# actuday6418/ray-tracer-s8

Measured on AMD Instinct MI355X. Metric: Mrays/sec @ 4K/8spp 1024-sphere, higher is better.
Workload: dtype f32

## Files before the change

ray_tracer_s8_amd/csrc/rt_kernel.hip.h:

```cpp
#pragma once
#include <hip/hip_runtime.h>
#include <type_traits>
#include <stdint.h>

#include "rt_consts.h"
#include "rt_cull.h"

namespace rtk {

#ifndef RT_MINWAVES
#define RT_MINWAVES 4
#endif
#ifndef RT_MINWAVES_TRAV
#define RT_MINWAVES_TRAV 4
#endif
#ifndef RT_MINWAVES_LTREE
#define RT_MINWAVES_LTREE 4
#endif
#ifndef RT_MINWAVES_CULL
#define RT_MINWAVES_CULL 5
#endif
#ifndef RT_STEPS_PER_CHECK_X
#define RT_STEPS_PER_CHECK_X 16
#endif
#ifndef RT_QUEUE_TAKE_MIN
#define RT_QUEUE_TAKE_MIN 4
#endif
#ifndef RT_BF2
#define RT_BF2 1
#endif
#ifndef RT_CULL_FLUSH_MIN
#define RT_CULL_FLUSH_MIN 1
#endif
#ifndef RT_MINWAVES_QTRAV
#define RT_MINWAVES_QTRAV 5
#endif
#ifndef RT_STEPS_PER_CHECK
#define RT_STEPS_PER_CHECK 8
#endif
#ifndef RT_STEPS_PER_CHECK_LTREE
#define RT_STEPS_PER_CHECK_LTREE 8
#endif
#ifndef RT_STEPS_PER_CHECK_Q
#define RT_STEPS_PER_CHECK_Q 16
#endif
#ifndef RT_LT_PARTIAL
#define RT_LT_PARTIAL 40
#endif
#ifndef RT_LT_EAGER
#define RT_LT_EAGER 12
#endif

constexpr uint32_t SLOT_FREE = 0x80000000u;
struct WaveQ {
    uint32_t cnt[SLOTS_MAX];
    uint32_t cost_acc[2];
    uint32_t cost_strip[2];
};
static_assert(sizeof(WaveQ) == 144, "WaveQ layout (rt_plan.h: LDS_LIMIT leaves 3 KiB of static LDS)");
constexpr uint32_t SLOT_UNIT_BITS = 13;
struct WaveStage {
    int left[STAGE_TILES + 1];
    uint32_t dst_lo[STAGE_TILES + 1], dst_hi[STAGE_TILES + 1];
};

struct StripDesc {
    uint64_t seed;
    uint8_t* rgb;
    float* f32;
    float* acc;
    uint32_t y0;
    uint32_t pad;
};

struct KParams {
    uint32_t W, H, Hs;
    uint32_t upp, depth;
    uint32_t spp_all, s_begin, gap;
    uint32_t acc_out;
    uint32_t n_sph, n_sph_pad;
    uint32_t n_tri;
    uint32_t chunk;
    uint32_t n_chunks;
    uint32_t flags;
    uint32_t path32;
    uint32_t lds_cand_off;
    uint32_t lds_path_off;
    uint32_t lds_rr_off;
    uint32_t lds_stack_off;
    uint32_t lds_cmp_off;
    uint32_t lds_stage_off;
    uint32_t n_strips;
    uint32_t tiles_x, tiles_per_strip;
    uint32_t tiles_total;
    uint32_t tiles_big;
    uint32_t sub_shift;
    uint32_t n_tiles;
    uint32_t n_slots;
    uint32_t grp;
    uint32_t grp_magic;
    uint32_t slot_stride;
    uint32_t commit_slots;
    uint32_t spp_magic;
    uint32_t slotu_magic;
    float* ring;
    float org[3], llc[3], hor[3], ver[3];
    float lens_radius, focus_distance;
    float lens_u[3], lens_v[3];
    float u_den, v_den;
    float t_min, t_max;
    float spp_f;
    float spp_rcp;
    const float4* geom_pk;
    const float4* geom_px;
    const float4* geom;
    const float4* mat;
    const float* emis;
    const float* tri;
    const float4* tri_box;
    const float4* trav;
    const uint4* travq;
    const float4* geom_r;
    float q_base[3], q_step[3], q_rstep[3];
    uint32_t root_ref;
    uint32_t maxl;
    uint32_t list16;
    uint32_t stack_lds;
    uint32_t ovf_stride;
    uint32_t* stack_ovf;
    const uint32_t* big;
    uint32_t n_big;
    float r_slack;
    float tri_k, tri_diag, tri_es, tri_e;
    uint32_t refill_eighths;
    uint32_t n_internal;
    uint32_t lds_node_off;
    const float4* bvh_nodes;
    const uint32_t* leaf_of;
    const uint32_t* world_rank;
    unsigned long long* strip_cost;
    unsigned long long* counters;
    unsigned long long* queue;
    StripDesc strips[MAX_BATCH];
    uint32_t plain;
};

struct V3 {
    float x, y, z;
};
__device__ __forceinline__ V3 mk(float x, float y, float z) { return V3{x, y, z}; }
__device__ __forceinline__ V3 operator+(V3 a, V3 b) { return {a.x + b.x, a.y + b.y, a.z + b.z}; }
__device__ __forceinline__ V3 operator-(V3 a, V3 b) { return {a.x - b.x, a.y - b.y, a.z - b.z}; }
__device__ __forceinline__ V3 operator*(float s, V3 a) { return {s * a.x, s * a.y, s * a.z}; }
__device__ __forceinline__ V3 operator*(V3 a, float s) { return {a.x * s, a.y * s, a.z * s}; }
template <class P>
__device__ __forceinline__ V3 lens_offset(const P& p, float x1, float x2) {
    return mk(x1 * p.lens_u[0] + x2 * p.lens_v[0], x1 * p.lens_u[1] + x2 * p.lens_v[1], x1 * p.lens_u[2] + x2 * p.lens_v[2]);
}
template <bool NEG_OK = false>
__device__ __forceinline__ float sqrt_rn(float x) {
#ifdef RT_IEEE_SQRT_PLAIN
    return __builtin_sqrtf(x);
#else
    const float r = __builtin_amdgcn_rsqf(x);
    float g = x * r, h = 0.5f * r;
    const float e = __builtin_fmaf(-h, g, 0.5f);
    g = __builtin_fmaf(g, e, g);
    h = __builtin_fmaf(h, e, h);
    const float dd = __builtin_fmaf(-g, g, x);
    float y = __builtin_fmaf(dd, h, g);
    const bool odd = ((__float_as_uint(x) & (NEG_OK ? 0x7fffffffu : 0xffffffffu)) - 0x0f800000u) >= (0x7f800000u - 0x0f800000u);
    if (__ballot(odd)) {
        if (odd) {
            asm volatile("" : "+v"(x));
            y = __builtin_sqrtf(x);
        }
    }
    return y;
#endif
}
#define RT_SQRT(x_) sqrt_rn(x_)
#define RT_SQRT_NEG_OK(x_) sqrt_rn<true>(x_)
#define RT_DIV(a_, b_) ((a_) / (b_))
#define RT_HOOK_LT_STEP_LOADS(nd_, ni_, lnodes_)
#define RT_HOOK_LT_STEP_ALU(p0_, p1_, p2_, p3_, oy_)
#define RT_HOOK_LT_STEP_END
#define RT_HOOK_Q_GATHER(t_ref_, cl_, travq_, n_internal_)
#ifdef RT_PROBES
#include "rt_probes.h"
#endif
__device__ __forceinline__ V3 operator/(V3 a, float s) { return {RT_DIV(a.x, s), RT_DIV(a.y, s), RT_DIV(a.z, s)}; }
__device__ __forceinline__ float dot(V3 a, V3 b) { return (a.x * b.x + a.y * b.y) + a.z * b.z; }
__device__ __forceinline__ float vlength(V3 a) { return RT_SQRT(dot(a, a)); }
__device__ __forceinline__ V3 normalize(V3 a) { return a / vlength(a); }
__device__ __forceinline__ bool try_normalize(V3 a, V3& out) {
    float rcp = RT_DIV(1.0f, RT_SQRT(dot(a, a)));
    if (rcp > 0.0f && rcp < __builtin_inff()) {
        out = a * rcp;
        return true;
    }
    return false;
}
__device__ __forceinline__ V3 normalize_or_zero(V3 a) {
// ... 279 lines not shown
    const float lcx = __builtin_fmaf(RT_Q(qa.x, 0), ig.x, cq.x), lcy = __builtin_fmaf(RT_Q(qa.x, 1), ig.y, cq.y), lcz = __builtin_fmaf(RT_Q(qa.y, 0), ig.z, cq.z);
    const float lhx = RT_Q(qa.y, 1), lhy = RT_Q(qa.z, 0), lhz = RT_Q(qa.z, 1);
    const float rcx = __builtin_fmaf(RT_Q(qa.w, 0), ig.x, cq.x), rcy = __builtin_fmaf(RT_Q(qa.w, 1), ig.y, cq.y), rcz = __builtin_fmaf(RT_Q(qb.x, 0), ig.z, cq.z);
    const float rhx = RT_Q(qb.x, 1), rhy = RT_Q(qb.y, 0), rhz = RT_Q(qb.y, 1);
#undef RT_Q
    lmin = __builtin_fmaxf(__builtin_fmaxf(__builtin_fmaf(-lhx, ax, lcx), __builtin_fmaf(-lhy, ay, lcy)), __builtin_fmaf(-lhz, az, lcz));
    lmax = __builtin_fminf(__builtin_fminf(__builtin_fmaf(lhx, ax, lcx), __builtin_fmaf(lhy, ay, lcy)), __builtin_fmaf(lhz, az, lcz));
    rmin_ = __builtin_fmaxf(__builtin_fmaxf(__builtin_fmaf(-rhx, ax, rcx), __builtin_fmaf(-rhy, ay, rcy)), __builtin_fmaf(-rhz, az, rcz));
    rmax_ = __builtin_fminf(__builtin_fminf(__builtin_fmaf(rhx, ax, rcx), __builtin_fmaf(rhy, ay, rcy)), __builtin_fmaf(rhz, az, rcz));
}

__device__ __forceinline__ float cull_bound(float best, V3 o, float r_slack) { return cull_bound(best, o.x, o.y, o.z, r_slack); }
__device__ __forceinline__ float cull_bound_tri(float best, V3 o, float k, float diag, float es, float e) {
    return cull_bound_tri(best, o.x, o.y, o.z, k, diag, es, e);
}

template <int ISECT, bool EXPANDED, int BS = BLOCK, bool STATS = false, bool TRIS = true>
__global__ __launch_bounds__(BS, (ISECT == 5 || ISECT == 6) ? RT_MINWAVES_LTREE : ISECT == 9 ? RT_MINWAVES_TRAV : ISECT >= 7 ? RT_MINWAVES_CULL : ISECT >= 3 ? RT_MINWAVES_QTRAV : ISECT == 2 ? RT_MINWAVES_TRAV : RT_MINWAVES) void rt_tile_kernel(const KParams p) {
    constexpr int BLOCK = BS;
    constexpr bool STREAMED = (ISECT == 1);
    constexpr bool TRAVERSE = (ISECT >= 2);
    constexpr bool QNODES = (ISECT == 3 || ISECT == 4 || ISECT == 7 || ISECT == 8);
    constexpr bool CULL = (ISECT == 6 || ISECT == 7 || ISECT == 8 || ISECT == 9);
    constexpr bool XNODES = (ISECT == 2 || ISECT == 9);
    constexpr bool CAPPED = (ISECT == 4 || ISECT == 8);
    constexpr bool LTREE = (ISECT == 5 || ISECT == 6);
    constexpr uint32_t LB = LTREE ? 0x8000u : LEAF_BIT;
    constexpr bool BFSTEP = LTREE;
    static_assert(TRIS || LTREE, "the sphere-only instantiation exists for the LDS-tree kernels");
    constexpr bool PLAIN_OK = LTREE;
    auto path32 = [&]() -> bool { return !LTREE && p.path32 != 0u; };
    const uint32_t ML = QNODES ? p.maxl : (uint32_t)MAXL_EXACT;
    extern __shared__ __attribute__((aligned(16))) unsigned char lds_raw[];
    __shared__ unsigned long long wg_tiles;
    __shared__ unsigned int wg_lock, wg_drained;
    __shared__ WaveQ wave_q[BS / 64];
    constexpr bool CAN_STAGE = (ISECT >= 1 && ISECT <= 4) || ISECT >= 7;
    __shared__ WaveStage wave_st[CAN_STAGE ? BS / 64 : 1];
    {
        uint32_t* z = reinterpret_cast<uint32_t*>(&wave_q[threadIdx.x >> 6]);
        if ((threadIdx.x & 63u) < SLOTS_MAX) wave_q[threadIdx.x >> 6].cnt[threadIdx.x & 63u] = SLOT_FREE;
        if ((threadIdx.x & 63u) == 0u) {
            wave_q[threadIdx.x >> 6].cost_acc[0] = wave_q[threadIdx.x >> 6].cost_acc[1] = 0u;
            wave_q[threadIdx.x >> 6].cost_strip[0] = wave_q[threadIdx.x >> 6].cost_strip[1] = 0xffffffffu;
        }
        (void)z;
        if (CAN_STAGE && (threadIdx.x & 63u) <= STAGE_TILES) wave_st[threadIdx.x >> 6].left[threadIdx.x & 63u] = -1;
    }
    if (threadIdx.x == 0) {
        wg_tiles = 0ull;
        wg_lock = 0u;
        wg_drained = 0u;
    }
    __syncthreads();
    float4* lgeom = reinterpret_cast<float4*>(lds_raw);
    const float* lgeomf = reinterpret_cast<const float*>(lds_raw);
    float* lrr = reinterpret_cast<float*>(lds_raw + p.lds_rr_off);
    const float4* __restrict__ gsrc = EXPANDED ? p.geom_px : p.geom_pk;
    uint16_t* lcand = reinterpret_cast<uint16_t*>(lds_raw + p.lds_cand_off);
    unsigned char* lpath = lds_raw + p.lds_path_off;

    const int tid = threadIdx.x;
    const int lane = tid & 63;
    const int tid16 = (tid & ~63) | ((tid & 31) << 1) | ((tid >> 5) & 1);

    if (ISECT == 0) {
        for (uint32_t i = tid; i < p.n_sph_pad; i += BLOCK) lgeom[i] = gsrc[i];
        if (EXPANDED)
            for (uint32_t i = tid; i < p.n_sph_pad; i += BLOCK) lrr[i] = p.geom[i].w;
        __syncthreads();
    }

    if (LTREE) {
        float* ln = reinterpret_cast<float*>(lds_raw + p.lds_node_off);
        const uint32_t r0 = lt_r0(p.n_internal);
        for (uint32_t n = tid; n <= p.n_internal; n += BLOCK) {
            float* q = ln + LNODE_DW * n;
            if (n < p.n_internal) {
                const float4 a0 = p.trav[4u * n], a1 = p.trav[4u * n + 1], a2 = p.trav[4u * n + 2], a3 = p.trav[4u * n + 3];
                auto ref16 = [r0](uint32_t r) { return (r & LEAF_BIT) ? (0x8000u | (r & 0x7fffu)) : r0 + r * (uint32_t)LNODE_DW; };
                q[0] = a0.x; q[1] = a1.x; q[2] = a0.x;   q[3] = a2.x; q[4] = a3.x; q[5] = a2.x;
                q[6] = a0.y; q[7] = a1.y; q[8] = a0.y;   q[9] = a2.y; q[10] = a3.y; q[11] = a2.y;
                q[12] = a0.z; q[13] = a1.z; q[14] = a0.z; q[15] = a2.z; q[16] = a3.z; q[17] = a2.z;
                q[18] = __uint_as_float(ref16(__float_as_uint(a0.w)) | (ref16(__float_as_uint(a1.w)) << 16));
            } else {
                const float qn = __builtin_nanf(""), inf = __builtin_inff();
                for (int i = 0; i < 18; i++) q[i] = qn;
                for (int a = 0; a < 3; a++) { q[6 * a] = -inf; q[6 * a + 1] = inf; q[6 * a + 2] = -inf; }
                q[18] = __uint_as_float((r0 + p.n_internal * (uint32_t)LNODE_DW) * 0x10001u);
            }
        }
        float* nanf_ = ln + LNODE_DW * (p.n_internal + 1u);
        for (uint32_t i = tid; i < p.n_sph + p.n_tri + (uint32_t)LNODE_DW; i += BLOCK) nanf_[i] = __builtin_nanf("");
        __syncthreads();
    }
    const float* const lnodes = reinterpret_cast<const float*>(lds_raw + p.lds_node_off) - (LTREE ? (int)lt_r0(p.n_internal) : 0);
    const V3 corg = mk(p.org[0], p.org[1], p.org[2]);
    const V3 llc = mk(p.llc[0], p.llc[1], p.llc[2]);
    const V3 hor = mk(p.hor[0], p.hor[1], p.hor[2]);
    const V3 ver = mk(p.ver[0], p.ver[1], p.ver[2]);
    const bool exact_scan = (p.flags & 1u) != 0;
    const bool use_bvh = (p.flags & 2u) == 0;
    const float KMf = 1.0f - 0x1p-17f;
    const v2f NKM = {-KMf, -KMf};

    const uint32_t wave = (uint32_t)tid >> 6;
#define wq wave_q[wave]
#define wst wave_st[CAN_STAGE ? wave : 0u]
    float* const ring = p.ring + (size_t)(blockIdx.x * (uint32_t)(BLOCK / 64) + wave) * ((size_t)p.n_slots * p.slot_stride * 3u);
    const uint32_t all_free = p.n_slots >= 32u ? 0xffffffffu : (1u << p.n_slots) - 1u;
    uint32_t freem = all_free;
    uint32_t cur_slot = 0;
    uint32_t tile_u = 0, tile_units = 0;
    uint32_t tile_x0 = 0, tile_row = 0, tile_yg = 0;
    uint32_t tile_meta = STAGE_TILES << 16;
    uint64_t tile_seed = 0;
    bool q_drained = false;
    bool have_unit = false, need_ray = false;
    uint32_t useq = 0;
    Rng rng = {0, 0, 0, 0};
    uint32_t depth_left = 0, k = 0;
    V3 o = mk(0, 0, 0), d = mk(0, 0, 0);
    bool bounce = false;
    V3 bn = mk(0, 0, 0);
    float brough = 0.f;
    using Cnt = typename std::conditional<(ISECT >= 2), uint32_t, unsigned long long>::type;
    Cnt n_seg = 0, n_cand = 0, n_fall = 0;
    Cnt n_int = 0;
    Hit h;
    h.idx = -1;
    h.dist = 0.f;
    h.t = 0.f;
    RayAux aux = ray_aux(mk(1.f, 1.f, 1.f), false);
    auto AUX = [&]() -> RayAux { return QNODES ? ray_aux(d, (p.flags & 8u) != 0) : aux; };
    auto far_bound = [&](float best) -> float {
        float b = cull_bound(best, o, p.r_slack);
        if (TRIS && (ISECT == 9 || ISECT == 6) && p.n_tri) b = __builtin_fmaxf(b, cull_bound_tri(best, o, p.tri_k, p.tri_diag, p.tri_es, p.tri_e));
        return b;
    };
    V3 td = mk(0, 0, 0);
    bool in_trav = false;
    uint32_t t_ref = 0, t_sp = 0, t_cnt = 0;
    uint32_t t_head = 0;
    V3 ig = mk(0, 0, 0), cq = mk(0, 0, 0);
    bool qfin = false;
    float t_far = __builtin_inff();
    uint32_t* lc32 = reinterpret_cast<uint32_t*>(lds_raw + p.lds_cand_off);
    uint32_t* lstack = reinterpret_cast<uint32_t*>(lds_raw + p.lds_stack_off);
    uint32_t sgx = 0, sgy = 0, sgz = 0;
    uint16_t* lc16 = reinterpret_cast<uint16_t*>(lds_raw + p.lds_cand_off);
    uint16_t* lstack16 = reinterpret_cast<uint16_t*>(lds_raw + p.lds_stack_off);

    if (BFSTEP) lstack16[tid16] = (uint16_t)(lt_r0(p.n_internal) + p.n_internal * (uint32_t)LNODE_DW);

    auto drain_counters = [&]() {
        const unsigned long long ws = wave_sum(n_seg), wc = wave_sum(n_cand), wf = wave_sum(n_fall);
        const unsigned long long wi = STATS ? wave_sum(n_int) : 0ull;
        if (lane == (int)__builtin_ctzll(__ballot(true))) {
            atomicAdd(&p.counters[0], ws);
            atomicAdd(&p.counters[1], wc);
            atomicAdd(&p.counters[2], wf);
            if (STATS) atomicAdd(&p.counters[3], wi);
        }
        n_seg = n_cand = n_fall = 0;
        n_int = 0;
    };
    const bool staging = CAN_STAGE && p.lds_stage_off != 0xffffffffu;
    unsigned char* const stage_base = lds_raw + (staging ? p.lds_stage_off + wave * (STAGE_TILES * STAGE_TILE_BYTES) : 0u);
    auto decode_tile = [&](uint32_t t, uint32_t& st, uint32_t& x0, uint32_t& row) {
        st = t / p.tiles_per_strip;
        const uint32_t rem = t - st * p.tiles_per_strip;
        row = rem / p.tiles_x;
        x0 = (rem - row * p.tiles_x) << 6;
    };
    auto div_spp = [&](uint32_t q) -> uint32_t { return p.spp_magic ? __umulhi(q, p.spp_magic) : q; };

    TDECL;
    for (;;) {
        WCOUNT(0);
        TSTAMP(5);
        TROUND;
        uint32_t px = 0, pyg = 0;
        if (freem != all_free) {
            __builtin_amdgcn_fence(__ATOMIC_ACQ_REL, "wavefront");
            const bool slot_done = (uint32_t)lane < SLOTS_MAX && (wq.cnt[cold<QNODES>(lane) & (int)(SLOTS_MAX - 1u)] & (SLOT_FREE | ((1u << SLOT_UNIT_BITS) - 1u))) == 0u;
            const uint32_t complete = (uint32_t)__ballot(slot_done);
            const uint32_t n_complete = (uint32_t)__builtin_popcount(complete);
            const bool issue_over = q_drained && tile_u == tile_units;
            if (n_complete >= p.commit_slots || (n_complete != 0u && ((uint32_t)__builtin_popcount(freem) < 2u || issue_over))) {
                WCOUNT(14);
                asm volatile("s_waitcnt vmcnt(0)" ::: "memory");
                auto commit_complete = [&](auto plain_tag) {
                    constexpr bool PLAIN = decltype(plain_tag)::value;
                    const uint32_t n_lanes = PLAIN ? p.n_slots : p.n_slots * p.grp;
                    for (uint32_t l0 = 0; l0 < n_lanes; l0 += 64u) {
                        const uint32_t L = l0 + (uint32_t)lane;
                        const uint32_t slot = (PLAIN || p.grp == 1u) ? L : __umulhi(L, p.grp_magic), g = PLAIN ? 0u : L - slot * p.grp;
                        const bool mine = slot < p.n_slots && ((complete >> (slot & 31u)) & 1u) != 0u;
                        if (__ballot(mine) == 0ull) continue;
                        uint32_t stg = STAGE_TILES, cstrip = 0;
                        bool fin = false;
                        uint32_t pin = 0;
                        if (mine) {
                            const float* sb = ring + __umul24(slot, p.slot_stride) * 3u;
                            const uint32_t hx = ring_load(reinterpret_cast<const uint32_t*>(sb) + 0);
                            const uint32_t hrow = ring_load(reinterpret_cast<const uint32_t*>(sb) + 1);
                            const uint32_t hmeta = ring_load(reinterpret_cast<const uint32_t*>(sb) + 2);
                            const float* r = sb + 3u + g * p.upp * 3u;
                            float sum_r = 0.f, sum_g = 0.f, sum_b = 0.f;
                            cstrip = hmeta & 0xffu;
                            if (!PLAIN && p.s_begin != 0u && g < ((hmeta >> 8) & 0xffu)) {
                                const float* a = p.strips[cstrip].acc + ((size_t)hrow * p.W + hx + g) * 3;
                                sum_r = a[0];
                                sum_g = a[1];
                                sum_b = a[2];
                            }
                            {
                                uint32_t i = 0;
                                auto batch = [&](auto cb_tag) {
                                    constexpr int CB = decltype(cb_tag)::value;
#pragma clang loop unroll(disable)
                                    for (; i + (uint32_t)CB <= p.upp; i += (uint32_t)CB) {
                                        LCOUNT(12);
                                        float c[3 * CB];
#pragma unroll
                                        for (int e = 0; e < 3 * CB; e++) c[e] = ring_load(r + e);
#pragma unroll
                                        for (int e = 0; e < CB; e++) {
                                            sum_r = sum_r + c[3 * e + 0];
                                            sum_g = sum_g + c[3 * e + 1];
                                            sum_b = sum_b + c[3 * e + 2];
                                        }
                                        r += 3 * CB;
                                    }
                                };
                                if (RT_COMMIT_BATCH > 4 && !QNODES) batch(std::integral_constant<int, RT_COMMIT_BATCH>{});
                                batch(std::integral_constant<int, 4>{});
#pragma clang loop unroll(disable)
                                for (; i < p.upp; i++) {
                                    LCOUNT(12);
                                    const float cr = ring_load(r + 0);
                                    const float cg = ring_load(r + 1);
                                    const float cb = ring_load(r + 2);
                                    sum_r = sum_r + cr;
                                    sum_g = sum_g + cg;
                                    sum_b = sum_b + cb;
                                    r += 3;
                                }
                            }
                            if (g < ((hmeta >> 8) & 0xffu)) {
                                float cr_, cg_, cb_;
                                if (PLAIN || p.spp_rcp != 0.0f) {
                                    cr_ = __builtin_sqrtf(sum_r * p.spp_rcp);
                                    cg_ = __builtin_sqrtf(sum_g * p.spp_rcp);
                                    cb_ = __builtin_sqrtf(sum_b * p.spp_rcp);
                                } else {
                                    cr_ = __builtin_sqrtf(sum_r / p.spp_f);
                                    cg_ = __builtin_sqrtf(sum_g / p.spp_f);
                                    cb_ = __builtin_sqrtf(sum_b / p.spp_f);
                                }
                                const uint32_t sidx = hmeta & 0xffu;
                                stg = (hmeta >> 16) & 0xffu;
                                const size_t oidx = ((size_t)hrow * p.W + hx + g) * 3;
                                if (!PLAIN && p.acc_out) {
                                    float* a = p.strips[sidx].acc;
                                    a[oidx + 0] = sum_r;
                                    a[oidx + 1] = sum_g;
                                    a[oidx + 2] = sum_b;
                                }
                                if (!CAN_STAGE || stg == STAGE_TILES) {
                                    uint8_t* orgb = p.strips[sidx].rgb;
                                    orgb[oidx + 0] = f32_as_u8(cr_ * 255.999f);
                                    orgb[oidx + 1] = f32_as_u8(cg_ * 255.999f);
                                    orgb[oidx + 2] = f32_as_u8(cb_ * 255.999f);
                                } else {
                                    uint8_t* sd = stage_base + stg * STAGE_TILE_BYTES + ((hx + g) & 63u) * 3u;
                                    sd[0] = f32_as_u8(cr_ * 255.999f);
                                    sd[1] = f32_as_u8(cg_ * 255.999f);
                                    sd[2] = f32_as_u8(cb_ * 255.999f);
                                    fin = true;
                                }
                                float* of = PLAIN ? nullptr : p.strips[sidx].f32;
                                if (of) {
                                    of[oidx + 0] = cr_;
                                    of[oidx + 1] = cg_;
                                    of[oidx + 2] = cb_;
                                }
                                (void)pin;
                            }
                        }
                        if (!PLAIN && p.strip_cost && mine && g == 0u) {
                            const uint32_t sg = wq.cnt[slot & (SLOTS_MAX - 1u)] >> SLOT_UNIT_BITS;
                            if (cstrip == wq.cost_strip[0]) (void)__hip_atomic_fetch_add(&wq.cost_acc[0], sg, __ATOMIC_RELAXED, __HIP_MEMORY_SCOPE_WAVEFRONT);
                            else if (cstrip == wq.cost_strip[1]) (void)__hip_atomic_fetch_add(&wq.cost_acc[1], sg, __ATOMIC_RELAXED, __HIP_MEMORY_SCOPE_WAVEFRONT);
                            else if (sg) atomicAdd(&p.strip_cost[(blockIdx.x % COST_COPIES) * MAX_BATCH + cstrip], (unsigned long long)sg);
                        }
                        if (CAN_STAGE && __ballot(fin)) {
                            __builtin_amdgcn_fence(__ATOMIC_ACQ_REL, "wavefront");
#pragma unroll
                            for (uint32_t k = 0; k < STAGE_TILES; k++) {
                                const unsigned long long mk = __ballot(fin && stg == k);
                                if (mk == 0ull) continue;
                                const int left = (int)uni((uint32_t)wst.left[k]) - (int)__builtin_popcountll(mk);
                                if (left == 0) {
                                    if (lane < (int)(STAGE_TILE_BYTES / 4)) {
                                        uint32_t* d32 = reinterpret_cast<uint32_t*>(((uintptr_t)uni(wst.dst_hi[k]) << 32) | uni(wst.dst_lo[k]));
// ... 81 lines not shown
                    tile_x0 = uni(tile_x0 + sub);
                    tile_row = uni(tile_row);
                    if (tile_x0 >= p.W) continue;
                    tile_yg = uni(p.strips[tstrip].y0 + tile_row);
                    tile_seed = p.strips[tstrip].seed + (((uint64_t)tile_yg * p.W + tile_x0) * p.spp_all + p.s_begin) * (4ull * PHI);
                    tile_seed = (uint64_t)uni((uint32_t)tile_seed) | ((uint64_t)uni((uint32_t)(tile_seed >> 32)) << 32);
                    const uint32_t npix = min(tw, p.W - tile_x0);
                    tile_units = uni(npix * p.upp);
                    tile_u = 0u;
                    uint32_t tstage = STAGE_TILES;
                    if (staging && npix == 64u) {
                        uint8_t* dst = p.strips[tstrip].rgb + ((size_t)tile_row * p.W + tile_x0) * 3;
                        if ((reinterpret_cast<uintptr_t>(dst) & 3u) == 0) {
                            __builtin_amdgcn_fence(__ATOMIC_ACQ_REL, "wavefront");
                            for (uint32_t k = 0; k < STAGE_TILES; k++)
                                if ((int)uni((uint32_t)wst.left[k]) < 0) {
                                    tstage = k;
                                    break;
                                }
                            if (tstage < STAGE_TILES && lane == 0) {
                                wst.left[tstage] = 64;
                                wst.dst_lo[tstage] = (uint32_t)reinterpret_cast<uintptr_t>(dst);
                                wst.dst_hi[tstage] = (uint32_t)(reinterpret_cast<uintptr_t>(dst) >> 32);
                            }
                            __builtin_amdgcn_fence(__ATOMIC_ACQ_REL, "wavefront");
                        }
                    }
                    tile_meta = uni(tstrip | (tstage << 16));
                }
                bool got = false;
                uint32_t tv = 0;
                bool stall = false;
                {
                    const unsigned long long mask = __ballot(need);
                    const uint32_t want = (uint32_t)__builtin_popcountll(mask);
                    const uint32_t U = p.slot_stride - 1u;
                    const uint32_t k_open = __umulhi(tile_u + U - 1u, p.slotu_magic);
                    const uint32_t n_free = (uint32_t)__builtin_popcount(freem);
                    const uint32_t slot_room = (k_open + n_free) * U - tile_u;
                    const uint32_t take = min(want, min(tile_units - tile_u, slot_room));
                    stall = take < want && take == slot_room;
                    const uint32_t n_new = __umulhi(tile_u + take + U - 1u, p.slotu_magic) - k_open;
                    const uint32_t rank = __builtin_amdgcn_mbcnt_hi((uint32_t)(mask >> 32), __builtin_amdgcn_mbcnt_lo((uint32_t)mask, 0u));
                    got = need && rank < take;
                    tv = tile_u + rank;
                    const uint32_t k = __umulhi(tv, p.slotu_magic);
                    const uint32_t unit = tv - __umul24(k, U);
                    uint32_t m = freem;
                    for (uint32_t i = 0; i + 1u < n_new; i++) m = k > k_open + i ? (m & (m - 1u)) : m;
                    const uint32_t slot = k >= k_open ? (uint32_t)__builtin_ctz(m | 0x80000000u) : cur_slot;
                    if (got) {
                        useq = (slot << 24) | unit;
                        if (unit == 0u) {
                            const uint32_t un = min(U, tile_units - tv);
                            wq.cnt[slot] = un;
                            uint32_t* hdr = reinterpret_cast<uint32_t*>(ring + __umul24(slot, p.slot_stride) * 3u);
                            hdr[0] = tile_x0 + __umul24(k, p.grp);
                            hdr[1] = tile_row;
                            hdr[2] = (tile_meta & 0xffu) | (div_spp(un) << 8) | (tile_meta & 0xff0000u);
                        }
                    }
                    tile_u = uni(tile_u + take);
                    if (n_new) {
                        uint32_t fm = freem;
                        for (uint32_t i = 0; i + 1u < n_new; i++) fm &= fm - 1u;
                        cur_slot = uni((uint32_t)__builtin_ctz(fm));
                        freem = uni(fm & (fm - 1u));
                    }
                }
                TSTAMP(7);
                if (got) {
                    WCOUNT(1);
                    LCOUNT(0);
                    const uint32_t j = div_spp(tv);
                    px = tile_x0 + j;
                    pyg = tile_yg;
                    rng = seed_state(tile_seed + (uint64_t)(tv + __umul24(j, p.gap)) * (4ull * PHI));
                    have_unit = true;
                    need_ray = true;
                    bounce = false;
                    need = false;
                }
                if (stall) { LCOUNT(14); break; }
            }
        }
        const bool active = have_unit;
        if (!active) { LCOUNT(13); }
        TSTAMP(0);
        if (active && need_ray) {
            float x1, x2, sm;
            WCOUNT(2);
            for (;;) {
                WCOUNT(3);
                LCOUNT(1);
                x1 = uniform_m1_1(rng);
                x2 = uniform_m1_1(rng);
                sm = x1 * x1 + x2 * x2;
                if (bounce ? !(sm >= 1.0f) : (sm <= 1.0f)) break;
            }
            V3 xdir, pre, fallback;
            LCOUNT(2);
            if (bounce) {
                LCOUNT(3);
                const float factor = 2.0f * RT_SQRT(1.0f - sm);
                const V3 us = mk(x1 * factor, x2 * factor, 1.0f - 2.0f * sm);
                const V3 diffuse_dir = us + bn;
                const V3 glossy_dir = d - (2.0f * dot(d, bn)) * bn;
                pre = diffuse_dir + brough * (glossy_dir - diffuse_dir);
                fallback = bn;
            } else {
                LCOUNT(4);
                const V3 offset = lens_offset(p, x1, x2);
                const float u = ((float)px + gen_range_01(rng)) / p.u_den;
                const float v = ((float)(p.H - pyg - 1) + gen_range_01(rng)) / p.v_den;
                const V3 dir0 = normalize_or_zero(llc + u * hor + v * ver - corg);
                const V3 d1 = normalize(dir0);
                const V3 focal_point = corg + p.focus_distance * d1;
                o = corg + offset;
                pre = focal_point - o;
                fallback = mk(0.f, 0.f, 0.f);
                depth_left = p.depth;
                k = 0;
            }
            if (!try_normalize(pre, xdir)) xdir = fallback;
            d = normalize(xdir);
            need_ray = false;
            bounce = false;
        }
        TSTAMP(1);
        const bool wave_busy = __ballot(active) != 0ull || freem != all_free || !q_drained || tile_u != tile_units;
        if (STREAMED) {
            if (!__syncthreads_or(wave_busy ? 1 : 0)) break;
        } else {
            if (!wave_busy) break;
        }

        if (active && !in_trav) {
            h.idx = -1;
            aux = ray_aux(d, (p.flags & 8u) != 0);
            if (!TRAVERSE) td = 2.0f * d;
            n_seg++;
            if (QNODES) {
                const V3 og = mk((o.x - p.q_base[0]) * p.q_rstep[0], (o.y - p.q_base[1]) * p.q_rstep[1], (o.z - p.q_base[2]) * p.q_rstep[2]);
                ig = mk(p.q_step[0] * aux.inv.x, p.q_step[1] * aux.inv.y, p.q_step[2] * aux.inv.z);
                cq = mk(-(og.x * ig.x), -(og.y * ig.y), -(og.z * ig.z));
                const float big = 0x1p100f, tiny = 0x1p-60f;
                const float ax = __builtin_fabsf(ig.x), ay = __builtin_fabsf(ig.y), az = __builtin_fabsf(ig.z);
                qfin = aux.finite && ax < big && ay < big && az < big && ax > tiny && ay > tiny && az > tiny &&
                       __builtin_fabsf(og.x) < 0x1p18f && __builtin_fabsf(og.y) < 0x1p18f && __builtin_fabsf(og.z) < 0x1p18f;
            }
            if (LTREE) {
                aux.finite = aux.finite && __builtin_fabsf(o.x) < __builtin_inff() && __builtin_fabsf(o.y) < __builtin_inff() &&
                             __builtin_fabsf(o.z) < __builtin_inff();
                sgx = aux.sx ? 1u : 0u;
                sgy = aux.sy ? 1u : 0u;
                sgz = aux.sz ? 1u : 0u;
            }
            if (CULL) {
                t_far = __builtin_inff();
                for (uint32_t j = 0; j < p.n_big; j++) {
                    const uint32_t prim = p.big[j];
                    float t;
                    bool hit;
                    if (!TRIS || prim < p.n_sph) {
                        const float4 g = RT_SPHERE_REC(p, prim);
                        hit = exact_sphere(o, 2.0f * d, mk(g.x, g.y, g.z), g.w, p.t_min, p.t_max, t);
                    } else {
                        hit = exact_triangle(o, d, p.tri + 9 * (size_t)(prim - p.n_sph), p.t_min, p.t_max, t);
                    }
                    if (hit)
                        consider_if<true>(h, (int)prim, o, d, t, [&]() { return bvh_reaches(p.bvh_nodes, p.leaf_of[prim], o, AUX()); }, p.leaf_of);
                }
                if (h.idx >= 0) t_far = far_bound(h.dist);
            }
            if (TRAVERSE) {
                t_ref = p.root_ref;
                t_sp = BFSTEP ? 1u : 0u;
                t_cnt = 0;
                in_trav = (p.n_sph + p.n_tri) > 0;
            }
        }
        if constexpr (TRAVERSE) {
            auto root_test = [&](uint32_t i) {
                    LCOUNT(6);
                    const uint32_t prim = LTREE ? (uint32_t)lc16[i * BLOCK + tid16] & 0x7fffu
                                          : p.list16 ? (uint32_t)lc16[i * BLOCK + tid16] : lc32[i * BLOCK + tid];
                    float t;
                    if (!TRIS || prim < p.n_sph) {
                        const float4 g = RT_SPHERE_REC(p, prim);
                        if (exact_sphere(o, 2.0f * d, mk(g.x, g.y, g.z), g.w, p.t_min, p.t_max, t)) {
                            if (QNODES)
                                consider_if<CULL>(h, (int)prim, o, d, t, [&]() {
                                    if (!qfin || (p.n_sph + p.n_tri) == 1) return true;
                                    const float4 s = at32(p.geom_r, prim);
                                    return intersects_aabb_finite(o, AUX(), make_float4(s.x - s.w, s.y - s.w, s.z - s.w, 0.f),
                                                                  make_float4(s.x + s.w, s.y + s.w, s.z + s.w, 0.f));
                                }, p.leaf_of);
                            else if (CULL)
                                consider<1>(h, (int)prim, o, d, t, aux, p.bvh_nodes, p.leaf_of);
                            else
                                consider<0>(h, (int)prim, o, d, t, aux, p.bvh_nodes, p.leaf_of);
                        }
                    } else {
                        if (exact_triangle(o, d, p.tri + 9 * (size_t)(prim - p.n_sph), p.t_min, p.t_max, t)) {
                            if (QNODES)
                                consider_if(h, (int)prim, o, d, t,
                                            [&]() { return !qfin || bvh_reaches(p.bvh_nodes, p.leaf_of[prim], o, AUX()); });
                            else if (CULL)
                                consider<1>(h, (int)prim, o, d, t, aux, p.bvh_nodes, p.leaf_of);
                            else
                                consider<0>(h, (int)prim, o, d, t, aux, p.bvh_nodes, p.leaf_of);
                        }
                    }
            };
            auto flush = [&]() {
                if (BFSTEP) n_cand += t_cnt - t_head;
#pragma clang loop unroll(disable)
                for (uint32_t i = BFSTEP ? t_head : 0u; i < t_cnt; i++) root_test(i);
                t_cnt = 0;
                if (BFSTEP) t_head = 0;
                if (CULL && h.idx >= 0) t_far = far_bound(h.dist);
            };
            auto flush_one = [&]() {
                n_cand++;
                root_test(t_head);
                t_head++;
                if (t_head == t_cnt) t_head = t_cnt = 0;
                if (CULL && h.idx >= 0) t_far = far_bound(h.dist);
            };

            constexpr bool COMPACT = XNODES;
            auto flush_c = [&](bool want) {
                const uint32_t cnt = want ? t_cnt : 0u;
                uint32_t excl = 0, total = 0;
#pragma unroll
                for (int b = 0; b < 4; b++) {
                    const unsigned long long m = __ballot(((cnt >> b) & 1u) != 0);
                    excl += (uint32_t)__builtin_amdgcn_mbcnt_hi((uint32_t)(m >> 32), __builtin_amdgcn_mbcnt_lo((uint32_t)m, 0u)) << b;
                    total += (uint32_t)__builtin_popcountll(m) << b;
                }
                const unsigned long long act = __ballot(true);
                const uint32_t n_act = (uint32_t)__builtin_popcountll(act);
                const uint32_t rank = (uint32_t)__builtin_amdgcn_mbcnt_hi((uint32_t)(act >> 32), __builtin_amdgcn_mbcnt_lo((uint32_t)act, 0u));
                uint32_t* const w_pref = reinterpret_cast<uint32_t*>(lds_raw + p.lds_cmp_off) + (tid >> 6) * 256;
                float* const w_dist = reinterpret_cast<float*>(w_pref + 64);
                float* const w_root = reinterpret_cast<float*>(w_pref + 128);
                uint32_t* const w_hit = w_pref + 192;
                w_pref[rank] = excl | ((uint32_t)lane << 16);
                __builtin_amdgcn_fence(__ATOMIC_ACQ_REL, "wavefront");
                int best_k = -1;
                float best_t = 0.f;
                auto own_prim = [&](uint32_t k) -> uint32_t {
                    return p.list16 ? (uint32_t)lc16[k * BLOCK + tid16] : lc32[k * BLOCK + tid];
                };
                for (uint32_t base = 0; base < total; base += n_act) {
                    const uint32_t j = base + rank;
                    const bool valid = j < total;
                    uint32_t R = 0, ent = w_pref[0];
                    if (valid) {
#pragma unroll
                        for (uint32_t stp = 32; stp > 0; stp >>= 1) {
                            const uint32_t c = R + stp;
                            if (c < n_act) {
                                const uint32_t e = w_pref[c];
                                if ((e & 0xffffu) <= j) { R = c; ent = e; }
                            }
                        }
                    }
                    const uint32_t L = ent >> 16, slot = j - (ent & 0xffffu);
                    const V3 ro = mk(__shfl(o.x, (int)L, 64), __shfl(o.y, (int)L, 64), __shfl(o.z, (int)L, 64));
                    const V3 rd = mk(__shfl(d.x, (int)L, 64), __shfl(d.y, (int)L, 64), __shfl(d.z, (int)L, 64));
                    bool hit = false;
                    float t = 0.f, dist = 0.f;
                    if (valid) {
                        LCOUNT(6);
                        const uint32_t ot = ((uint32_t)tid & ~63u) | L;
                        const uint32_t ot16 = (ot & ~63u) | ((ot & 31u) << 1) | ((ot >> 5) & 1u);
                        const uint32_t prim = p.list16 ? (uint32_t)lc16[slot * BLOCK + ot16] : lc32[slot * BLOCK + ot];
                        if (prim < p.n_sph) {
                            const float4 g = RT_SPHERE_REC(p, prim);
                            hit = exact_sphere(ro, 2.0f * rd, mk(g.x, g.y, g.z), g.w, p.t_min, p.t_max, t);
                        } else {
                            hit = exact_triangle(ro, rd, p.tri + 9 * (size_t)(prim - p.n_sph), p.t_min, p.t_max, t);
                        }
                        if (hit) {
                            const V3 pp = ro + t * rd;
                            dist = vlength(pp - ro);
                        }
                    }
                    w_dist[rank] = dist;
                    w_root[rank] = t;
                    w_hit[rank] = hit ? 1u : 0u;
                    __builtin_amdgcn_fence(__ATOMIC_ACQ_REL, "wavefront");
                    if (cnt) {
                        const uint32_t k0 = excl > base ? excl : base, k1 = min(excl + cnt, base + n_act);
#pragma clang loop unroll(disable)
                        for (uint32_t k = k0; k < k1; k++) {
                            if (!w_hit[k - base]) continue;
                            const float dk = w_dist[k - base];
                            bool take = best_k < 0 ? (h.idx < 0 || h.dist > dk) : (h.dist > dk);
                            if (CULL && !take && h.dist == dk && (best_k >= 0 || h.idx >= 0)) {
                                const uint32_t cur = best_k >= 0 ? own_prim((uint32_t)best_k) : (uint32_t)h.idx;
                                take = p.leaf_of[own_prim(k - excl)] < p.leaf_of[cur];
                            }
                            if (take) {
                                h.dist = dk;
                                best_k = (int)(k - excl);
                                best_t = w_root[k - base];
                            }
                        }
                    }
                    __builtin_amdgcn_fence(__ATOMIC_ACQ_REL, "wavefront");
                }
                if (best_k >= 0) {
                    h.idx = (int)own_prim((uint32_t)best_k);
                    h.t = best_t;
                }
                if (want) t_cnt = 0;
                if (CULL && want && h.idx >= 0) t_far = far_bound(h.dist);
            };
            auto push = [&](uint32_t v) {
                if (LTREE) lstack16[t_sp * BLOCK + tid16] = (uint16_t)v;
                else if (!CAPPED || t_sp < p.stack_lds) lstack[t_sp * BLOCK + tid] = v;
                else p.stack_ovf[(size_t)(t_sp - p.stack_lds) * p.ovf_stride + (blockIdx.x * BLOCK + tid)] = v;
                t_sp++;
            };
            auto pop = [&]() -> uint32_t {
                --t_sp;
                if (LTREE) return (uint32_t)lstack16[t_sp * BLOCK + tid16];
                if (!CAPPED || t_sp < p.stack_lds) return lstack[t_sp * BLOCK + tid];
                return p.stack_ovf[(size_t)(t_sp - p.stack_lds) * p.ovf_stride + (blockIdx.x * BLOCK + tid)];
            };
            if constexpr (BFSTEP) {
            const uint32_t DONE = lt_r0(p.n_internal) + p.n_internal * (uint32_t)LNODE_DW;
            constexpr int STEPS = RT_STEPS_PER_CHECK_LTREE;
            static_assert(MAXL_LTREE > STEPS, "the leaf list must take a block of appends");
            constexpr uint32_t SLOT = (uint32_t)BLOCK * 2u;
            typedef __attribute__((address_space(3))) unsigned char lds_byte;
            typedef __attribute__((address_space(3))) uint16_t lds_u16;
            const uint32_t lds0 = (uint32_t)(uintptr_t)(lds_byte*)lds_raw;
            const uint32_t stack0_a = lds0 + p.lds_stack_off + (uint32_t)tid16 * 2u;
            const uint32_t list0_m = lds0 + p.lds_cand_off + (uint32_t)tid16 * 2u - SLOT;
            uint32_t top_a = 0, cnt_m = 0;
            auto lds16 = [&](uint32_t a) -> lds_u16& { return *(lds_u16*)(uintptr_t)a; };
            auto step = [&](auto slow_tag) {
                constexpr bool SLOW = decltype(slow_tag)::value;
                static_assert(SLOT == 0x800u, "leaf flag 0x8000 >> 4 must be one slot");
                const uint32_t leaf_slot = (t_ref >> 4) & SLOT;
                const uint32_t ni = t_ref;
                if (STATS) n_int += (ni < DONE) ? 1u : 0u;
                const uint32_t top = (uint32_t)lds16(top_a);
                WCOUNT(5);
                LCOUNT(5);
                lds16(cnt_m + SLOT) = (uint16_t)t_ref;
                const float* __restrict__ nd = lnodes + ni;
                const float* __restrict__ fx = nd + sgx;
                const float* __restrict__ fy = nd + 6 + sgy;
                const float* __restrict__ fz = nd + 12 + sgz;
                const float p0 = fx[0], p1 = fx[1], p2 = fx[3], p3 = fx[4], p4 = fy[0], p5 = fy[1], p6 = fy[3], p7 = fy[4];
                const float p8 = fz[0], p9 = fz[1], p10 = fz[3], p11 = fz[4];
                const uint32_t refs = __float_as_uint(nd[18]);
                RT_HOOK_LT_STEP_LOADS(nd, ni, lnodes);
                __builtin_amdgcn_sched_barrier(0);
                RT_HOOK_LT_STEP_ALU(p0, p1, p2, p3, o.y);
                const float lxn = (p0 - o.x) * aux.inv.x, lxf = (p1 - o.x) * aux.inv.x;
                const float rxn = (p2 - o.x) * aux.inv.x, rxf = (p3 - o.x) * aux.inv.x;
                const float lyn = (p4 - o.y) * aux.inv.y, lyf = (p5 - o.y) * aux.inv.y;
                const float ryn = (p6 - o.y) * aux.inv.y, ryf = (p7 - o.y) * aux.inv.y;
                const float lzn = (p8 - o.z) * aux.inv.z, lzf = (p9 - o.z) * aux.inv.z;
                const float rzn = (p10 - o.z) * aux.inv.z, rzf = (p11 - o.z) * aux.inv.z;
                bool hl, hr;
                float le, re;
                if (SLOW) {
                    le = rmax(rmax(rmax(lxn, lyn), lzn), 0.0f);
                    re = rmax(rmax(rmax(rxn, ryn), rzn), 0.0f);
                    hl = le <= rmin(rmin(lxf, lyf), lzf);
                    hr = re <= rmin(rmin(rxf, ryf), rzf);
                } else {
                    le = __builtin_fmaxf(__builtin_fmaxf(__builtin_fmaxf(lxn, lyn), lzn), 0.0f);
                    re = __builtin_fmaxf(__builtin_fmaxf(__builtin_fmaxf(rxn, ryn), rzn), 0.0f);
                    hl = le <= __builtin_fminf(__builtin_fminf(lxf, lyf), lzf);
                    hr = re <= __builtin_fminf(__builtin_fminf(rxf, ryf), rzf);
                }
                uint32_t cl = refs & 0xffffu, cr = refs >> 16;
                if (CULL) {
                    hl = hl && le <= t_far;
                    hr = hr && re <= t_far;
                    const bool swp = hl && hr && re < le;
                    const uint32_t c0 = cl;
                    cl = swp ? cr : cl;
                    cr = swp ? c0 : cr;
                }
                lds16(top_a + SLOT) = (uint16_t)cr;
                const bool any = hl || hr;
                t_ref = any ? (hl ? cl : cr) : top;
                uint32_t delta = any ? 0u : 0u - SLOT;
                delta = (hl && hr) ? SLOT : delta;
                asm volatile("" : "+v"(delta));
                top_a += delta;
                if (SLOW) top_a = max(top_a, stack0_a);
                cnt_m += leaf_slot;
                RT_HOOK_LT_STEP_END;
            };
            for (;;) {
                const uint32_t walking = (uint32_t)__builtin_popcountll(__ballot(in_trav));
                const uint32_t live = (uint32_t)__builtin_popcountll(__ballot(active));
                if (walking == 0 || (walking * 8 <= live * p.refill_eighths && walking < live)) break;
                if (in_trav && t_cnt > p.maxl - (uint32_t)STEPS) flush();
                if (RT_LT_PARTIAL < 64) {
                    const bool pend = t_cnt > t_head;
                    if ((int)__builtin_popcountll(__ballot(pend)) >= RT_LT_PARTIAL ||
                        (CULL && (int)__builtin_popcountll(__ballot(pend && h.idx < 0)) >= RT_LT_EAGER)) {
                        if (pend) flush_one();
                    }
                }
                const bool slow = __ballot(in_trav && !aux.finite) != 0;
                if (in_trav) {
                    top_a = stack0_a + (t_sp - 1u) * SLOT;
                    cnt_m = list0_m + t_cnt * SLOT;
                    if (slow) {
#pragma unroll
                        for (int rep = 0; rep < STEPS; rep++) step(std::true_type{});
                    } else {
#pragma unroll
                        for (int rep = 0; rep < STEPS; rep++) step(std::false_type{});
                    }
                    t_sp = (top_a + SLOT - stack0_a) / SLOT;
                    t_cnt = (cnt_m - list0_m) / SLOT;
                    in_trav = t_ref != DONE;
                }
            }
            } else {
            for (;;) {
                const uint32_t walking = (uint32_t)__builtin_popcountll(__ballot(in_trav));
                const uint32_t live = (uint32_t)__builtin_popcountll(__ballot(active));
                if (walking == 0 || (walking * 8 <= live * p.refill_eighths && walking < live)) break;
#ifndef RT_FLUSH_INLINE
                if (COMPACT && p.lds_cmp_off != 0xffffffffu) {
                    const bool want = in_trav && (t_cnt == ML || (CULL && t_cnt >= (uint32_t)RT_CULL_FLUSH_MIN && h.idx < 0));
                    if (__ballot(want)) flush_c(want);
                } else
                if (in_trav && (t_cnt == ML || (CULL && t_cnt >= (uint32_t)RT_CULL_FLUSH_MIN && h.idx < 0))) flush();
#endif
                constexpr bool BF2 = (RT_BF2 != 0) && (XNODES || QNODES);
                if (BF2 && !__ballot(in_trav && !(QNODES ? qfin : aux.finite))) {
#pragma unroll
                    for (int rep = 0; rep < (QNODES ? RT_STEPS_PER_CHECK_Q : RT_STEPS_PER_CHECK_X); rep++)
                    if (in_trav) {
                        WCOUNT(5);
                        LCOUNT(5);
                        const bool is_leaf = (t_ref & LEAF_BIT) != 0;
                        if (STATS) n_int += is_leaf ? 0u : 1u;
                        const uint32_t tsl = t_sp - (t_sp ? 1u : 0u);
                        uint32_t top = lstack[(CAPPED ? min(tsl, p.stack_lds - 1u) : tsl) * BLOCK + tid];
                        bool hl, hr;
                        float le = 0.f, re = 0.f;
                        uint32_t c0, c1;
                        if constexpr (QNODES) {
                        const uint4* __restrict__ nq = reinterpret_cast<const uint4*>(reinterpret_cast<const char*>(p.travq) + ((is_leaf ? 0u : t_ref) << 5));
                        uint4 qa = nq[0], qb = nq[1];
                        asm volatile("" : "+v"(qb.x), "+v"(qb.y), "+v"(qb.z), "+v"(qb.w));
                        float lmin, lmax, rmin_, rmax_;
                        qslabs(qa, qb, ig, cq, lmin, lmax, rmin_, rmax_);
                        le = __builtin_fmaxf(lmin, 0.0f);
                        re = __builtin_fmaxf(rmin_, 0.0f);
                        hl = le <= (CULL ? __builtin_fminf(lmax, t_far) : lmax);
                        hr = re <= (CULL ? __builtin_fminf(rmax_, t_far) : rmax_);
                        c0 = qb.z;
                        c1 = qb.w;
                        } else {
                        const float4* __restrict__ nd = reinterpret_cast<const float4*>(reinterpret_cast<const char*>(p.trav) + ((is_leaf ? 0u : t_ref) << 6));
                        const float4 n0 = nd[0], n1 = nd[1], n2 = nd[2], n3 = nd[3];
                        if (CULL) {
                            float lmin, lmax, rmin_, rmax_;
                            slabs_finite(o, aux, n0, n1, lmin, lmax);
                            slabs_finite(o, aux, n2, n3, rmin_, rmax_);
                            le = __builtin_fmaxf(lmin, 0.0f);
                            re = __builtin_fmaxf(rmin_, 0.0f);
                            hl = le <= lmax && le <= t_far;
                            hr = re <= rmax_ && re <= t_far;
                        } else {
                            hl = intersects_aabb_finite(o, aux, n0, n1);
                            hr = intersects_aabb_finite(o, aux, n2, n3);
                        }
                        c0 = __float_as_uint(n0.w);
                        c1 = __float_as_uint(n1.w);
                        }
                        hl = hl && !is_leaf;
                        hr = hr && !is_leaf;
                        const bool both = hl && hr, any = hl || hr;
                        const bool swp = CULL && both && re < le;
                        const uint32_t cl = swp ? c1 : c0, cr = swp ? c0 : c1;
                        if (!CAPPED || t_sp < p.stack_lds) lstack[t_sp * BLOCK + tid] = cr;
                        else if (both) p.stack_ovf[(size_t)(t_sp - p.stack_lds) * p.ovf_stride + (blockIdx.x * BLOCK + tid)] = cr;
                        const bool can = t_cnt < ML, app = is_leaf && can, stall = is_leaf && !can;
                        if (app) {
                            if (p.list16) lc16[t_cnt * BLOCK + tid16] = (uint16_t)t_ref;
                            else lc32[t_cnt * BLOCK + tid] = t_ref & ~LEAF_BIT;
                        }
                        t_cnt += app ? 1u : 0u;
                        n_cand += app ? 1u : 0u;
                        const bool pop_ = !any && !stall, empty = t_sp == 0;
                        if (CAPPED && pop_ && t_sp > p.stack_lds)
                            top = p.stack_ovf[(size_t)(t_sp - 1u - p.stack_lds) * p.ovf_stride + (blockIdx.x * BLOCK + tid)];
                        t_ref = stall ? t_ref : any ? (hl ? cl : cr) : top;
                        in_trav = !(pop_ && empty);
                        t_sp = t_sp + (both ? 1u : 0u) - ((pop_ && !empty) ? 1u : 0u);
                    }
                } else
#if defined(RT_ROLL_STEPS) || RT_BF2
#pragma clang loop unroll(disable)
#else
#pragma unroll
#endif
                for (int rep = 0; rep < (QNODES ? RT_STEPS_PER_CHECK_Q : RT_STEPS_PER_CHECK); rep++)
                if (in_trav) {
                    WCOUNT(5);
                    LCOUNT(5);
                    if (t_ref & LB) {
#ifdef RT_FLUSH_INLINE
                        if (t_cnt == ML) flush();
#else
                        if (t_cnt == ML) continue;
#endif
                        if (p.list16) lc16[t_cnt * BLOCK + tid16] = (uint16_t)t_ref;
                        else lc32[t_cnt * BLOCK + tid] = t_ref & ~LEAF_BIT;
                        t_cnt++;
                        n_cand++;
                        if (t_sp == 0) {
                            in_trav = false;
                        } else {
                            t_ref = pop();
                        }
                    } else {
                        bool hl, hr;
                        uint32_t cl, cr;
                        if (STATS) n_int++;
                        if (QNODES) {
                            const uint4* __restrict__ nq = reinterpret_cast<const uint4*>(reinterpret_cast<const char*>(p.travq) + (t_ref << 5));
                            uint4 qa = nq[0], qb = nq[1];
                            asm volatile("" : "+v"(qb.x), "+v"(qb.y), "+v"(qb.z), "+v"(qb.w));
                            cl = qb.z;
                            cr = qb.w;
                            RT_HOOK_Q_GATHER(t_ref, cl, p.travq, p.n_internal);
                            if (qfin) {
                                float lmin, lmax, rmin_, rmax_;
                                qslabs(qa, qb, ig, cq, lmin, lmax, rmin_, rmax_);
                                if (CULL) {
                                    const float le = __builtin_fmaxf(lmin, 0.0f), re = __builtin_fmaxf(rmin_, 0.0f);
                                    hl = le <= __builtin_fminf(lmax, t_far);
                                    hr = re <= __builtin_fminf(rmax_, t_far);
                                    if (hl && hr && re < le) {
                                        const uint32_t t = cl;
                                        cl = cr;
                                        cr = t;
                                    }
                                } else {
                                    hl = __builtin_fmaxf(lmin, 0.0f) <= lmax;
                                    hr = __builtin_fmaxf(rmin_, 0.0f) <= rmax_;
                                }
                            } else {
                                const float4* __restrict__ nd = reinterpret_cast<const float4*>(reinterpret_cast<const char*>(p.trav) + (t_ref << 6));
                                const RayAux ax = AUX();
                                hl = intersects_aabb(o, ax, nd[0], nd[1]);
                                hr = intersects_aabb(o, ax, nd[2], nd[3]);
                            }
                        } else {
                            const float4* __restrict__ nd = reinterpret_cast<const float4*>(reinterpret_cast<const char*>(p.trav) + (t_ref << 6));
                            const float4 n0 = nd[0], n1 = nd[1], n2 = nd[2], n3 = nd[3];
                            if (aux.finite) {
                                hl = intersects_aabb_finite(o, aux, n0, n1);
                                hr = intersects_aabb_finite(o, aux, n2, n3);
                            } else {
                                hl = intersects_aabb(o, aux, n0, n1);
                                hr = intersects_aabb(o, aux, n2, n3);
                            }
                            cl = __float_as_uint(n0.w);
                            cr = __float_as_uint(n1.w);
                        }
                        if (hl) {
                            if (hr) push(cr);
// ... 286 lines not shown
```

Before: 16090.

## Keep LTREE traversal state as LDS byte addresses and hoist per-loop ballots

Traversal stack and leaf-list state is kept as LDS byte addresses (top_a, cnt_m, head_m) across the whole ray lifetime, so the per-iteration conversion to and from slot indices goes away. Flush and flush_one walk the list by address. Sign offsets are pre-scaled to bytes, and the stack delta is computed branch-free. The live-lane count, refill threshold and non-finite mask are hoisted out of the loop, and the walking mask comes from t_ref != DONE. This saves ALU and ballot work per traversal step, at the cost of more live registers and more complex state invariants.

```diff
diff --git a/ray_tracer_s8_amd/csrc/rt_kernel.hip.h b/ray_tracer_s8_amd/csrc/rt_kernel.hip.h
--- a/ray_tracer_s8_amd/csrc/rt_kernel.hip.h
+++ b/ray_tracer_s8_amd/csrc/rt_kernel.hip.h
@@ -49,6 +49,18 @@
 #endif
 #ifndef RT_LT_EAGER
 #define RT_LT_EAGER 12
+#endif
+#ifndef RT_R6_STEP1
+#define RT_R6_STEP1 1
+#endif
+#ifndef RT_R6_ADDR
+#define RT_R6_ADDR 1
+#endif
+#ifndef RT_R6_DELTA
+#define RT_R6_DELTA 1
+#endif
+#ifndef RT_R6_HEAD
+#define RT_R6_HEAD 1
 #endif
 
 constexpr uint32_t SLOT_FREE = 0x80000000u;
@@ -634,6 +646,16 @@
     uint16_t* lstack16 = reinterpret_cast<uint16_t*>(lds_raw + p.lds_stack_off);
 
     if (BFSTEP) lstack16[tid16] = (uint16_t)(lt_r0(p.n_internal) + p.n_internal * (uint32_t)LNODE_DW);
+    constexpr bool ADDR = BFSTEP && (RT_R6_ADDR != 0);
+    static_assert(!ADDR || sizeof(WaveQ) * (BS / 64) >= (size_t)BLOCK * 2u, "list0_m = lds0 + ... - SLOT must not wrap");
+    constexpr uint32_t SLOT = (uint32_t)BLOCK * 2u;
+    typedef __attribute__((address_space(3))) unsigned char lds_byte;
+    typedef __attribute__((address_space(3))) uint16_t lds_u16;
+    const uint32_t lds0 = (uint32_t)(uintptr_t)(lds_byte*)lds_raw;
+    const uint32_t stack0_a = lds0 + p.lds_stack_off + (uint32_t)tid16 * 2u;
+    const uint32_t list0_m = lds0 + p.lds_cand_off + (uint32_t)tid16 * 2u - SLOT;
+    uint32_t top_a = 0, cnt_m = list0_m, head_m = list0_m;
+    auto lds16 = [&](uint32_t a) -> lds_u16& { return *(lds_u16*)(uintptr_t)a; };
 
     auto drain_counters = [&]() {
         const unsigned long long ws = wave_sum(n_seg), wc = wave_sum(n_cand), wf = wave_sum(n_fall);
@@ -1021,9 +1043,9 @@
             if (LTREE) {
                 aux.finite = aux.finite && __builtin_fabsf(o.x) < __builtin_inff() && __builtin_fabsf(o.y) < __builtin_inff() &&
                              __builtin_fabsf(o.z) < __builtin_inff();
-                sgx = aux.sx ? 1u : 0u;
-                sgy = aux.sy ? 1u : 0u;
-                sgz = aux.sz ? 1u : 0u;
+                sgx = aux.sx ? (ADDR ? 4u : 1u) : 0u;
+                sgy = aux.sy ? (ADDR ? 4u : 1u) : 0u;
+                sgz = aux.sz ? (ADDR ? 4u : 1u) : 0u;
             }
             if (CULL) {
                 t_far = __builtin_inff();
@@ -1044,15 +1066,21 @@
             }
             if (TRAVERSE) {
                 t_ref = p.root_ref;
+                if (ADDR) {
+                    top_a = stack0_a;
+                    cnt_m = list0_m;
+                } else {
                 t_sp = BFSTEP ? 1u : 0u;
                 t_cnt = 0;
+                }
                 in_trav = (p.n_sph + p.n_tri) > 0;
             }
         }
         if constexpr (TRAVERSE) {
             auto root_test = [&](uint32_t i) {
                     LCOUNT(6);
-                    const uint32_t prim = LTREE ? (uint32_t)lc16[i * BLOCK + tid16] & 0x7fffu
+                    const uint32_t prim = ADDR ? (uint32_t)lds16(i + SLOT) & 0x7fffu
+                                          : LTREE ? (uint32_t)lc16[i * BLOCK + tid16] & 0x7fffu
                                           : p.list16 ? (uint32_t)lc16[i * BLOCK + tid16] : lc32[i * BLOCK + tid];
                     float t;
                     if (!TRIS || prim < p.n_sph) {
@@ -1083,6 +1111,14 @@
                     }
             };
             auto flush = [&]() {
+                if (ADDR) {
+                    n_cand += (cnt_m - head_m) / SLOT;
+#pragma clang loop unroll(disable)
+                    for (uint32_t a = head_m; a < cnt_m; a += SLOT) root_test(a);
+                    cnt_m = head_m = list0_m;
+                    if (CULL && h.idx >= 0) t_far = far_bound(h.dist);
+                    return;
+                }
                 if (BFSTEP) n_cand += t_cnt - t_head;
 #pragma clang loop unroll(disable)
                 for (uint32_t i = BFSTEP ? t_head : 0u; i < t_cnt; i++) root_test(i);
@@ -1092,9 +1128,15 @@
             };
             auto flush_one = [&]() {
                 n_cand++;
+                if (ADDR) {
+                    root_test(head_m);
+                    head_m += SLOT;
+                    if (head_m == cnt_m) head_m = cnt_m = list0_m;
+                } else {
                 root_test(t_head);
                 t_head++;
                 if (t_head == t_cnt) t_head = t_cnt = 0;
+                }
                 if (CULL && h.idx >= 0) t_far = far_bound(h.dist);
             };
 
@@ -1204,14 +1246,6 @@
             const uint32_t DONE = lt_r0(p.n_internal) + p.n_internal * (uint32_t)LNODE_DW;
             constexpr int STEPS = RT_STEPS_PER_CHECK_LTREE;
             static_assert(MAXL_LTREE > STEPS, "the leaf list must take a block of appends");
-            constexpr uint32_t SLOT = (uint32_t)BLOCK * 2u;
-            typedef __attribute__((address_space(3))) unsigned char lds_byte;
-            typedef __attribute__((address_space(3))) uint16_t lds_u16;
-            const uint32_t lds0 = (uint32_t)(uintptr_t)(lds_byte*)lds_raw;
-            const uint32_t stack0_a = lds0 + p.lds_stack_off + (uint32_t)tid16 * 2u;
-            const uint32_t list0_m = lds0 + p.lds_cand_off + (uint32_t)tid16 * 2u - SLOT;
-            uint32_t top_a = 0, cnt_m = 0;
-            auto lds16 = [&](uint32_t a) -> lds_u16& { return *(lds_u16*)(uintptr_t)a; };
             auto step = [&](auto slow_tag) {
                 constexpr bool SLOW = decltype(slow_tag)::value;
                 static_assert(SLOT == 0x800u, "leaf flag 0x8000 >> 4 must be one slot");
@@ -1223,9 +1257,12 @@
                 LCOUNT(5);
                 lds16(cnt_m + SLOT) = (uint16_t)t_ref;
                 const float* __restrict__ nd = lnodes + ni;
-                const float* __restrict__ fx = nd + sgx;
-                const float* __restrict__ fy = nd + 6 + sgy;
-                const float* __restrict__ fz = nd + 12 + sgz;
+                auto plane = [&](const float* q, uint32_t sg) -> const float* {
+                    return ADDR ? reinterpret_cast<const float*>(reinterpret_cast<const char*>(q) + sg) : q + sg;
+                };
+                const float* __restrict__ fx = plane(nd, sgx);
+                const float* __restrict__ fy = plane(nd + 6, sgy);
+                const float* __restrict__ fz = plane(nd + 12, sgz);
                 const float p0 = fx[0], p1 = fx[1], p2 = fx[3], p3 = fx[4], p4 = fy[0], p5 = fy[1], p6 = fy[3], p7 = fy[4];
                 const float p8 = fz[0], p9 = fz[1], p10 = fz[3], p11 = fz[4];
                 const uint32_t refs = __float_as_uint(nd[18]);
@@ -1263,39 +1300,60 @@
                 lds16(top_a + SLOT) = (uint16_t)cr;
                 const bool any = hl || hr;
                 t_ref = any ? (hl ? cl : cr) : top;
+#if RT_R6_DELTA
+                uint32_t delta = (hl ? 0u : 0u - SLOT) + (hr ? SLOT : 0u);
+#else
                 uint32_t delta = any ? 0u : 0u - SLOT;
                 delta = (hl && hr) ? SLOT : delta;
+#endif
                 asm volatile("" : "+v"(delta));
                 top_a += delta;
                 if (SLOW) top_a = max(top_a, stack0_a);
                 cnt_m += leaf_slot;
                 RT_HOOK_LT_STEP_END;
             };
+            constexpr bool HEAD = RT_R6_HEAD != 0;
+            if (HEAD && !in_trav) t_ref = DONE;
+            const uint32_t live_r = (uint32_t)__builtin_popcountll(__ballot(active));
+            const uint32_t refill_r = live_r * p.refill_eighths;
+            const unsigned long long nonfinite_r = __ballot(!aux.finite);
             for (;;) {
-                const uint32_t walking = (uint32_t)__builtin_popcountll(__ballot(in_trav));
-                const uint32_t live = (uint32_t)__builtin_popcountll(__ballot(active));
-                if (walking == 0 || (walking * 8 <= live * p.refill_eighths && walking < live)) break;
-                if (in_trav && t_cnt > p.maxl - (uint32_t)STEPS) flush();
+                const unsigned long long walk_m = HEAD ? __ballot(t_ref != DONE) : __ballot(in_trav);
+                uint32_t walking = (uint32_t)__builtin_popcountll(walk_m);
+                if (HEAD) asm("" : "+s"(walking));
+                const uint32_t live = HEAD ? live_r : (uint32_t)__builtin_popcountll(__ballot(active));
+                if (walking == 0 || (walking * 8 <= (HEAD ? refill_r : live * p.refill_eighths) && walking < live)) break;
+                if (in_trav && (ADDR ? cnt_m - list0_m > (p.maxl - (uint32_t)STEPS) * SLOT : t_cnt > p.maxl - (uint32_t)STEPS)) flush();
                 if (RT_LT_PARTIAL < 64) {
-                    const bool pend = t_cnt > t_head;
+                    const bool pend = ADDR ? cnt_m > head_m : t_cnt > t_head;
                     if ((int)__builtin_popcountll(__ballot(pend)) >= RT_LT_PARTIAL ||
                         (CULL && (int)__builtin_popcountll(__ballot(pend && h.idx < 0)) >= RT_LT_EAGER)) {
                         if (pend) flush_one();
                     }
                 }
-                const bool slow = __ballot(in_trav && !aux.finite) != 0;
+                const bool slow = HEAD ? (walk_m & nonfinite_r) != 0ull : __ballot(in_trav && !aux.finite) != 0;
                 if (in_trav) {
+                    if (!ADDR) {
                     top_a = stack0_a + (t_sp - 1u) * SLOT;
                     cnt_m = list0_m + t_cnt * SLOT;
+                    }
                     if (slow) {
+#if RT_R6_STEP1
+                        asm volatile("; slow block" ::: "memory");
+#endif
 #pragma unroll
                         for (int rep = 0; rep < STEPS; rep++) step(std::true_type{});
                     } else {
+#if RT_R6_STEP1
+                        asm volatile("; fast block" ::: "memory");
+#endif
 #pragma unroll
                         for (int rep = 0; rep < STEPS; rep++) step(std::false_type{});
                     }
+                    if (!ADDR) {
                     t_sp = (top_a + SLOT - stack0_a) / SLOT;
                     t_cnt = (cnt_m - list0_m) / SLOT;
+                    }
                     in_trav = t_ref != DONE;
                 }
             }
```

Result: faster. 16440 (median of 6 runs) (+2.2%).
